# nnanhuang/S3Gaussian

Hardware: AMD Instinct MI355X
Metric: train_iters_per_sec (higher is better)
Workload: dtype f32

## Files before the change

### include/s3g_raster.h

```cpp
#ifndef S3G_RASTER_H
#define S3G_RASTER_H

#include <stddef.h>
#include <stdint.h>

#ifdef __cplusplus
extern "C" {
#endif

#define S3G_OK 0
#define S3G_ERR_INVALID_ARG 1
#define S3G_ERR_HIP 2
#define S3G_ERR_ALLOC 3
#define S3G_ERR_PREFILTERED 4

typedef void* (*s3g_resize_fn)(void* user, size_t bytes);

typedef struct s3g_raster_inputs {
  int P;
  int D;
  int M;
  int width, height;
  const float* background;
  const float* means3D;
// ... 14 lines not shown

int s3g_raster_forward(const s3g_raster_inputs* in,
                       s3g_resize_fn geometry_buffer, void* geometry_user,
                       s3g_resize_fn binning_buffer, void* binning_user,
                       s3g_resize_fn image_buffer, void* image_user,
                       float* out_color, float* out_depth, int* radii,
                       int* num_rendered, void* stream );

int s3g_raster_forward_reuse(const s3g_raster_inputs* in, int R, const void* geometry_arena, const void* binning_arena,
                             void* image_arena, float* out_color, float* out_depth, void* stream);

int s3g_raster_forward_decompose(const s3g_raster_inputs* in, int R, const void* geometry_arena, const void* binning_arena,
                                 const void* image_arena, const uint8_t* is_dynamic, const long long* class_counts,
                                 float* out_color_d, float* out_depth_d,
                                 float* out_color_s, float* out_depth_s, void* stream);

int s3g_raster_forward2(const s3g_raster_inputs* in, const float* colors2,
                        s3g_resize_fn geometry_buffer, void* geometry_user,
                        s3g_resize_fn binning_buffer, void* binning_user,
                        s3g_resize_fn image_buffer, void* image_user,
                        float* out_color, float* out_depth, float* out_color2, int* radii,
                        int* num_rendered, void* stream );

typedef struct s3g_raster_async {
  uint32_t capacity_instances;
  uint32_t capacity_slots;
  uint32_t sort_lds_keys;
  int long_lists;
  void* geometry_arena;
  void* binning_arena;
  void* image_arena;
  uint32_t* status_device;
  uint32_t* status_host;
  int forward_only;
  uint32_t* sticky_device;
  void* status_event;
} s3g_raster_async;
int s3g_raster_arena_bytes(int P, int width, int height, uint32_t capacity_instances, uint32_t capacity_slots,
                           size_t* geometry_bytes, size_t* binning_bytes, size_t* image_bytes);
int s3g_raster_forward_async(const s3g_raster_inputs* in, const float* colors2, const s3g_raster_async* async_,
                             float* out_color, float* out_depth, float* out_color2, int* radii, void* stream);

size_t s3g_raster_backward_workspace_bytes(int P, int R);
int s3g_raster_backward(const s3g_raster_inputs* in, int R, const int* radii,
                        const void* geometry_arena, const void* binning_arena, const void* image_arena,
                        void* workspace,
                        const float* dL_dpix, const float* dL_dpix_depth,
                        float* dL_dmean2D, float* dL_dconic, float* dL_dopacity, float* dL_dcolor,
                        float* dL_ddepth, float* dL_dmean3D, float* dL_dcov3D, float* dL_dsh,
                        float* dL_dscale, float* dL_drot, void* stream);

size_t s3g_raster_backward2_workspace_bytes(int P, int R);
int s3g_raster_backward2(const s3g_raster_inputs* in, const float* colors2, int R, const int* radii,
                         const void* geometry_arena, const void* binning_arena, const void* image_arena,
                         void* workspace,
                         const float* dL_dpix, const float* dL_dpix_depth, const float* dL_dpix2,
                         float* dL_dmean2D, float* dL_dconic, float* dL_dopacity, float* dL_dcolor, float* dL_dcolor2,
                         float* dL_ddepth, float* dL_dmean3D, float* dL_dcov3D, float* dL_dscale, float* dL_drot,
                         void* stream);

typedef struct s3g_densify_accum {
  float* xyz_gradient_accum;
  float* denom;
  float* max_radii2D;
} s3g_densify_accum;
int s3g_raster_backward_accum(const s3g_raster_inputs* in, int R, const int* radii,
                              const void* geometry_arena, const void* binning_arena, const void* image_arena,
                              void* workspace, const float* dL_dpix, const float* dL_dpix_depth,
                              float* dL_dmean2D, float* dL_dconic, float* dL_dopacity, float* dL_dcolor,
                              float* dL_ddepth, float* dL_dmean3D, float* dL_dcov3D, float* dL_dsh,
                              float* dL_dscale, float* dL_drot, const s3g_densify_accum* dens, void* stream);
int s3g_raster_backward2_accum(const s3g_raster_inputs* in, const float* colors2, int R, const int* radii,
                               const void* geometry_arena, const void* binning_arena, const void* image_arena,
                               void* workspace, const float* dL_dpix, const float* dL_dpix_depth, const float* dL_dpix2,
                               float* dL_dmean2D, float* dL_dconic, float* dL_dopacity, float* dL_dcolor,
                               float* dL_dcolor2, float* dL_ddepth, float* dL_dmean3D, float* dL_dcov3D,
                               float* dL_dscale, float* dL_drot, const s3g_densify_accum* dens, void* stream);

void s3g_raster_set_exact_cull(int on);
int s3g_raster_get_exact_cull(void);

int s3g_raster_set_backward_wave_bounds(int on);

int s3g_raster_set_bin_band(int tiles);

int s3g_mark_visible(int P, const float* means3D, const float* viewmatrix, const float* projmatrix,
                     uint8_t* present, void* stream);

enum {
  S3G_PROFILE_BLEND_FORWARD = 0,
  S3G_PROFILE_BLEND_BACKWARD = 1,
  S3G_PROFILE_HEXPLANE_FORWARD = 2,
  S3G_PROFILE_HEXPLANE_BACKWARD_POINT = 3,
  S3G_PROFILE_HEXPLANE_SCATTER = 4,
  S3G_PROFILE_MLP_FORWARD = 5,
  S3G_PROFILE_MLP_BACKWARD = 6,
  S3G_PROFILE_MLP_WGRAD = 7,
  S3G_PROFILE_ADAM = 8,
  S3G_PROFILE_DEFORM_INFER = 9,
  S3G_PROFILE_IDS = 10
};
void s3g_profile_enable(int on);
int s3g_profile_read(int id, double* total_ms, double* total_instances, double* total_pixels);

const char* s3g_last_error(void);

int s3g_abi_version(void);

#ifdef __cplusplus
}
#endif
#endif
```

### s3gaussian_amd/_lib.py

```python
from __future__ import annotations

import ctypes as C
import os
import subprocess

_HERE = os.path.dirname(os.path.abspath(__file__))
LIB_PATH = os.environ.get("S3G_LIB_PATH") or os.path.join(_HERE, "lib", "libs3g.so")
CSRC_DIR = os.path.join(_HERE, "csrc")

ABI_VERSION = 16

RESIZE_FN = C.CFUNCTYPE(C.c_void_p, C.c_void_p, C.c_size_t)


class RasterInputs(C.Structure):
    _fields_ = [
        ("P", C.c_int), ("D", C.c_int), ("M", C.c_int), ("width", C.c_int), ("height", C.c_int),
        ("background", C.c_void_p), ("means3D", C.c_void_p), ("shs", C.c_void_p), ("colors_precomp", C.c_void_p),
        ("opacities", C.c_void_p), ("scales", C.c_void_p), ("scale_modifier", C.c_float), ("rotations", C.c_void_p),
        ("cov3D_precomp", C.c_void_p), ("viewmatrix", C.c_void_p), ("projmatrix", C.c_void_p), ("cam_pos", C.c_void_p),
        ("tan_fovx", C.c_float), ("tan_fovy", C.c_float), ("prefiltered", C.c_int), ("debug", C.c_int),
    ]


# ... 39 lines not shown
    L.s3g_raster_backward.restype = C.c_int
    L.s3g_raster_backward.argtypes = [C.POINTER(RasterInputs), C.c_int] + [vp] * 18
    L.s3g_raster_backward_workspace_bytes.restype = C.c_size_t
    L.s3g_raster_backward_workspace_bytes.argtypes = [C.c_int, C.c_int]
    L.s3g_raster_forward2.restype = C.c_int
    L.s3g_raster_forward2.argtypes = [C.POINTER(RasterInputs), vp, RESIZE_FN, vp, RESIZE_FN, vp, RESIZE_FN, vp, vp, vp, vp, vp,
                                      C.POINTER(C.c_int), vp]
    L.s3g_raster_set_exact_cull.restype = None
    L.s3g_raster_set_exact_cull.argtypes = [C.c_int]
    L.s3g_raster_get_exact_cull.restype = C.c_int
    L.s3g_raster_backward2.restype = C.c_int
    L.s3g_raster_backward2.argtypes = [C.POINTER(RasterInputs), vp, C.c_int] + [vp] * 19
    L.s3g_raster_backward2_workspace_bytes.restype = C.c_size_t
    L.s3g_raster_backward2_workspace_bytes.argtypes = [C.c_int, C.c_int]
    L.s3g_mark_visible.restype = C.c_int
    L.s3g_mark_visible.argtypes = [C.c_int, vp, vp, vp, vp, vp]
    L.s3g_raster_forward_decompose.restype = C.c_int
    L.s3g_raster_forward_decompose.argtypes = [C.POINTER(RasterInputs), C.c_int] + [vp] * 10
    L.s3g_raster_backward_accum.restype = C.c_int
    L.s3g_raster_backward_accum.argtypes = [C.POINTER(RasterInputs), C.c_int] + [vp] * 17 + [C.POINTER(DensifyAccum), vp]
    L.s3g_raster_backward2_accum.restype = C.c_int
    L.s3g_raster_backward2_accum.argtypes = [C.POINTER(RasterInputs), vp, C.c_int] + [vp] * 18 + [C.POINTER(DensifyAccum), vp]
    L.s3g_raster_arena_bytes.restype = C.c_int
    L.s3g_raster_arena_bytes.argtypes = [C.c_int, C.c_int, C.c_int, C.c_uint32, C.c_uint32] + [C.POINTER(C.c_size_t)] * 3
    L.s3g_raster_forward_async.restype = C.c_int
    L.s3g_raster_forward_async.argtypes = [C.POINTER(RasterInputs), vp, C.POINTER(RasterAsync), vp, vp, vp, vp, vp]
    L.s3g_densify_stats.restype = C.c_int
    L.s3g_densify_stats.argtypes = [C.c_int, vp, C.c_int, vp, vp, vp, vp, vp, vp]
    L.s3g_densify_stats_guarded.restype = C.c_int
    L.s3g_densify_stats_guarded.argtypes = [C.c_int, vp, C.c_int, vp, vp, vp, vp, vp, vp, vp]
    _lib = L
    return L


def _bind_fast_paths():
    import torch
    raw = getattr(torch._C, "_cuda_getCurrentRawStream", None)
    cur = getattr(torch._C, "_cuda_getDevice", None)
    return torch, raw, cur


_torch = _raw_stream = _cur_device = None


def stream_ptr() -> int:
    global _torch, _raw_stream, _cur_device
    if _torch is None:
        _torch, _raw_stream, _cur_device = _bind_fast_paths()
    if _raw_stream is not None and _cur_device is not None:
        return _raw_stream(_cur_device())
    return _torch.cuda.current_stream().cuda_stream


class _NullContext:
    __slots__ = ()

    def __enter__(self):
        return None

    def __exit__(self, *exc):
        return False


_NULL = _NullContext()


def on_device(dev):
    global _torch, _raw_stream, _cur_device
    if _torch is None:
        _torch, _raw_stream, _cur_device = _bind_fast_paths()
    if _cur_device is not None and getattr(dev, "index", None) is not None and _cur_device() == dev.index:
        return _NULL
    return _torch.cuda.device(dev)


def check(code: int) -> None:
    if code != 0:
        msg = lib().s3g_last_error().decode("utf-8", "replace")
        if code == 1:
            raise Exception(msg)
        raise RuntimeError(f"libs3g error {code}: {msg}")


EXPORTED_SYMBOLS = ["s3g_raster_forward", "s3g_raster_forward_reuse", "s3g_raster_forward_decompose", "s3g_raster_forward2", "s3g_raster_forward_async", "s3g_raster_arena_bytes", "s3g_adam_step_guarded", "s3g_raster_backward", "s3g_raster_backward_workspace_bytes", "s3g_raster_backward2", "s3g_raster_backward2_workspace_bytes", "s3g_hexplane_forward_workspace_bytes", "s3g_knn_workspace_bytes", "s3g_knn_mean_dist2", "s3g_hexplane_forward", "s3g_hexplane_backward", "s3g_hexplane_backward_algo", "s3g_hexplane_backward_workspace_bytes", "s3g_hexplane_backward_scratch_rows", "s3g_hexplane_debug_walk_mask", "s3g_hexplane_set_deterministic", "s3g_hexplane_get_deterministic", "s3g_hexplane_sort_state_words", "s3g_profile_enable", "s3g_profile_read", "s3g_ssim_forward", "s3g_ssim_backward", "s3g_plane_regulation", "s3g_scale_unless_one", "s3g_pixel_losses_forward", "s3g_pixel_losses_combine", "s3g_pixel_losses_backward", "s3g_photometric_forward", "s3g_photometric_backward", "s3g_glue_forward", "s3g_glue_backward", "s3g_deform_mlp_forward", "s3g_deform_mlp_backward", "s3g_deform_mlp_backward_ordered", "s3g_deform_mlp_wgrad_partial_bytes", "s3g_deform_mlp_stash_bytes", "s3g_deform_mlp_pack_bytes", "s3g_deform_mlp_set_arithmetic", "s3g_deform_mlp_get_arithmetic", "s3g_deform_infer", "s3g_deform_infer_split", "s3g_deform_infer_workspace_bytes", "s3g_adam_step", "s3g_densify_stats", "s3g_densify_stats_guarded", "s3g_density_count_words", "s3g_density_classify_densify", "s3g_density_classify_prune", "s3g_density_scan", "s3g_density_apply", "s3g_density_reset_opacity", "s3g_image_metrics_workspace_bytes", "s3g_image_metrics", "s3g_scene_flow_workspace_bytes", "s3g_scene_flow_colors", "s3g_frame_workspace_bytes", "s3g_frame_tiles", "s3g_split_count_words", "s3g_split_workspace_bytes", "s3g_split_classify", "s3g_split_mask_offsets", "s3g_split_pack_rows", "s3g_lpips_weights_bytes", "s3g_lpips_pack_weights", "s3g_lpips_workspace_bytes", "s3g_lpips", "s3g_lpips_vgg_weights_bytes", "s3g_lpips_vgg_pack_weights", "s3g_lpips_vgg_workspace_bytes", "s3g_lpips_vgg", "s3g_raster_backward_accum", "s3g_raster_backward2_accum", "s3g_mark_visible", "s3g_raster_set_exact_cull", "s3g_raster_get_exact_cull", "s3g_raster_set_bin_band", "s3g_raster_set_backward_wave_bounds", "s3g_last_error", "s3g_abi_version"]
```

### s3gaussian_amd/csrc/raster_backward.hip

```cpp
#include "geom_math.hpp"
#include "raster_dev.hpp"

namespace s3g {

template <int CTRL, int ROW_MASK>
__device__ __forceinline__ float dpp_add(float v) {
  const int t = __builtin_amdgcn_update_dpp(0, __float_as_int(v), CTRL, ROW_MASK, 0xf, false);
  return v + __int_as_float(t);
}
__device__ __forceinline__ float wave_sum_lane63(float v) {
  v = dpp_add<0x111, 0xf>(v);
  v = dpp_add<0x112, 0xf>(v);
  v = dpp_add<0x114, 0xf>(v);
  v = dpp_add<0x118, 0xf>(v);
  v = dpp_add<0x142, 0xa>(v);
  v = dpp_add<0x143, 0xc>(v);
  return v;
}

__device__ __forceinline__ float row_sum_lane15(float v) {
  v = dpp_add<0x111, 0xf>(v);
  v = dpp_add<0x112, 0xf>(v);
  v = dpp_add<0x114, 0xf>(v);
  v = dpp_add<0x118, 0xf>(v);
  asm volatile("" : "+v"(v));
  return v;
}

#define S3G_DPP_SET(dst, src, ctrl, bank) \
  asm volatile("v_add_f32_dpp %0, %1, %1 " ctrl " row_mask:0xf bank_mask:" bank : "=v"(dst) : "v"(src))
#define S3G_DPP_ACC(dst, src, ctrl, bank) \
  asm volatile("v_add_f32_dpp %0, %1, %1 " ctrl " row_mask:0xf bank_mask:" bank : "+v"(dst) : "v"(src))
#define S3G_DPP_SELF(dst, ctrl) asm volatile("v_add_f32_dpp %0, %0, %0 " ctrl " row_mask:0xf bank_mask:0xf" : "+v"(dst))
template <int NV>
__device__ __forceinline__ void row_transpose_reduce(const float* v , float* q ) {
  static_assert(NV > 8 && NV <= 16, "values per visit");
  float r[8];
  asm volatile("s_nop 1");
#pragma unroll
  for (int i = 0; i < 8; i++) {
    S3G_DPP_SET(r[i], v[i], "row_ror:8", "0x3");
    if (i + 8 < NV) S3G_DPP_ACC(r[i], v[i + 8], "row_ror:8", "0xc");
  }
  asm volatile("s_nop 1");
#pragma unroll
  for (int i = 0; i < 4; i++) {
    S3G_DPP_SET(q[i], r[i], "row_half_mirror", "0x5");
    S3G_DPP_ACC(q[i], r[i + 4], "row_half_mirror", "0xa");
  }
  asm volatile("s_nop 1");
#pragma unroll
  for (int i = 0; i < 4; i++) S3G_DPP_SELF(q[i], "quad_perm:[1,0,3,2]");
  asm volatile("s_nop 1");
#pragma unroll
  for (int i = 0; i < 4; i++) S3G_DPP_SELF(q[i], "quad_perm:[2,3,0,1]");
}

template <int NX>
__global__ void __launch_bounds__(256)
blend_backward_kernel(int W, int H, int gx, int tiles, const uint2* __restrict__ ranges,
                      const uint32_t* __restrict__ tile_hi, const uint32_t* __restrict__ point_list,
                      const float* __restrict__ bg, const float2* __restrict__ means2D,
                      const float4* __restrict__ conic_opacity, const float* __restrict__ colors,
                      const float* __restrict__ depths, const float* __restrict__ final_Ts,
                      const uint32_t* __restrict__ n_contrib, const float* __restrict__ dL_dpixels,
                      const float* __restrict__ dL_dpixel_depths, float* __restrict__ records ,
                      const float* __restrict__ colors2, const float* __restrict__ dL_dpixels2, int wave_bounds) {
  constexpr uint32_t BATCH = 32;
  constexpr int NR = NX ? NREC + 4 : NREC;
  constexpr int SLOTS = 16;
  __shared__ StagedGaussian sg[BATCH];
  __shared__ float4 sg2[NX ? BATCH : 1];
  constexpr int NV = NX ? NREC + 3 : NREC;
  constexpr int RS = BATCH + 1;
  constexpr int SLOT_FLOATS = NV * RS;
  __shared__ float acc[SLOTS][SLOT_FLOATS];
  __shared__ uint32_t visited[4];

  const uint32_t tile = xcd_swizzle(blockIdx.x, gridDim.x);
  if (tile >= (uint32_t)tiles) return;
  const uint2 rg = ranges[tile];
  const uint32_t hi = tile_hi[tile] - rg.x;
  if (hi == 0) return;
  const int tx = tile % gx, ty = tile / gx;
  const int tid = threadIdx.x, lane = tid & 63, wave = tid >> 6;
  const int px = tx * TILE_X + (tid & 15), py = ty * TILE_Y + (tid >> 4);
  const bool inside = px < W && py < H;
  const float pxf = (float)px, pyf = (float)py;
  const size_t pix = (size_t)py * W + px, N = (size_t)H * W;

  const float T_final = inside ? final_Ts[pix] : 0.f;
  const uint32_t last_contributor = inside ? n_contrib[pix] : 0u;
  uint32_t whi = last_contributor;
  for (int off = 32; off >= 1; off >>= 1) whi = max(whi, (uint32_t)__shfl_xor((int)whi, off));
  whi = wave_bounds ? __builtin_amdgcn_readfirstlane(whi) : hi;
  float gr = 0.f, gg = 0.f, gb = 0.f, gd = 0.f;
  if (inside) {
    gr = dL_dpixels[pix];
    gg = dL_dpixels[N + pix];
    gb = dL_dpixels[2 * N + pix];
    gd = dL_dpixel_depths[pix];
  }
  float g2r = 0.f, g2g = 0.f, g2b = 0.f;
  if (NX && inside) {
    g2r = dL_dpixels2[pix];
    g2g = dL_dpixels2[N + pix];
    g2b = dL_dpixels2[2 * N + pix];
  }
  float bg_dot = bg[0] * gr + bg[1] * gg + bg[2] * gb;
  if (NX) bg_dot += bg[0] * g2r + bg[1] * g2g + bg[2] * g2b;

  float T = T_final;
  float ar = 0.f, ag = 0.f, ab = 0.f, ad = 0.f;
  float last_alpha = 0.f, lr = 0.f, lg = 0.f, lb = 0.f, ld = 0.f;
  float a2r = 0.f, a2g = 0.f, a2b = 0.f, l2r = 0.f, l2g = 0.f, l2b = 0.f;

  for (uint32_t done_cnt = 0; done_cnt < hi; done_cnt += BATCH) {
    const uint32_t cnt = min(BATCH, hi - done_cnt);
    __syncthreads();
    if ((uint32_t)tid < cnt) {
      const uint32_t pos = hi - 1 - (done_cnt + tid);
      const uint32_t id = point_list[rg.x + pos];
      const float2 mm = means2D[id];
      const float4 co = conic_opacity[id];
      StagedGaussian s;
      s.a = make_float4(mm.x, mm.y, -0.5f * LOG2E * co.x, -LOG2E * co.y);
      s.b = make_float4(-0.5f * LOG2E * co.z, co.w, depths[id], colors[3 * (size_t)id]);
      s.c = make_float4(colors[3 * (size_t)id + 1], colors[3 * (size_t)id + 2], 0.f, 0.f);
      sg[tid] = s;
      if (NX) sg2[tid] = make_float4(colors2[3 * (size_t)id], colors2[3 * (size_t)id + 1], colors2[3 * (size_t)id + 2], 0.f);
    }
    __syncthreads();

    const uint32_t j0 = hi - done_cnt > whi ? hi - done_cnt - whi : 0u;
    uint32_t vis = 0u;
    for (uint32_t j = j0; j < cnt; j++) {
      const uint32_t pos = hi - 1 - (done_cnt + j);
      bool valid = pos < last_contributor;
      const float4 A = sg[j].a;
      const float4 B = sg[j].b;
      const float dx = A.x - pxf, dy = A.y - pyf;
      const float q = gaussian_exponent2(dx, dy, A.z, A.w, B.x);
      const float G = __builtin_amdgcn_exp2f(q);
      const float alpha = fminf(0.99f, B.y * G);
      valid = valid && !(q > 0.f) && !(alpha < 1.0f / 255.0f);
      if (__ballot(valid) == 0ull) continue;
      vis |= 1u << j;

      float p_r = 0.f, p_g = 0.f, p_b = 0.f, p_d = 0.f, s0 = 0.f, sx = 0.f, sy = 0.f, sxx = 0.f, sxy = 0.f, syy = 0.f;
      float p2_r = 0.f, p2_g = 0.f, p2_b = 0.f;
      if (valid) {
        const float4 Cc = sg[j].c;
        const float cr = B.w, cg = Cc.x, cb = Cc.y, cd = B.z;
        const float rcp = __builtin_amdgcn_rcpf(1.f - alpha);
        T = T * rcp;
        const float w = alpha * T;
        const float one_m_la = 1.f - last_alpha;
        ar = last_alpha * lr + one_m_la * ar;
        ag = last_alpha * lg + one_m_la * ag;
        ab = last_alpha * lb + one_m_la * ab;
        ad = last_alpha * ld + one_m_la * ad;
        lr = cr; lg = cg; lb = cb; ld = cd;
        float dL_dalpha = (cr - ar) * gr + (cg - ag) * gg + (cb - ab) * gb + (cd - ad) * gd;
        if (NX) {
          const float4 C2 = sg2[j];
          a2r = last_alpha * l2r + one_m_la * a2r;
          a2g = last_alpha * l2g + one_m_la * a2g;
          a2b = last_alpha * l2b + one_m_la * a2b;
          l2r = C2.x; l2g = C2.y; l2b = C2.z;
          dL_dalpha += (C2.x - a2r) * g2r + (C2.y - a2g) * g2g + (C2.z - a2b) * g2b;
          p2_r = w * g2r; p2_g = w * g2g; p2_b = w * g2b;
        }
        dL_dalpha *= T;
        last_alpha = alpha;
        dL_dalpha += (-T_final * rcp) * bg_dot;
        p_r = w * gr; p_g = w * gg; p_b = w * gb; p_d = w * gd;
        const float v = dL_dalpha * G;
        const float vx = v * dx, vy = v * dy;
        s0 = v; sx = vx; sy = vy; sxx = vx * dx; sxy = vx * dy; syy = vy * dy;
      }
      const float vals[13] = {p_r, p_g, p_b, p_d, s0, sx, sy, sxx, sxy, syy, p2_r, p2_g, p2_b};
      float q4[4];
      row_transpose_reduce<NV>(vals, q4);
      if ((lane & 3) == 0) {
        float* aw = &acc[wave * 4 + (lane >> 4)][(lane & 12) * RS + j];
#pragma unroll
        for (int i = 0; i < 4; i++)
          if ((lane & 12) + i < NV) aw[i * RS] = q4[i];
      }
    }
    if (lane == 0) visited[wave] = vis;
    __syncthreads();
    const uint32_t g = (uint32_t)tid % BATCH, k = (uint32_t)tid / BATCH;
    if (k < NR / 2 && g < cnt) {
      uint32_t seen[4];
#pragma unroll
      for (int w = 0; w < 4; w++) seen[w] = 0u - ((visited[w] >> g) & 1u);
      auto slot = [&](int q, uint32_t v) { return __uint_as_float(__float_as_uint(acc[q][v * RS + g]) & seen[q / 4]); };
      const uint32_t v1 = 2 * k + 1 < (uint32_t)NV ? 2 * k + 1 : 2 * k;
      float lo = slot(0, 2 * k), hi2 = slot(0, v1);
#pragma unroll
      for (int q = 1; q < SLOTS; q++) {
        lo += slot(q, 2 * k);
        hi2 += slot(q, v1);
      }
      const uint32_t pos = hi - 1 - (done_cnt + g);
      float2* rec = reinterpret_cast<float2*>(records + (size_t)(rg.x + pos) * NR);
      rec[k] = make_float2(lo, 2 * k + 1 < (uint32_t)NV ? hi2 : 0.f);
    }
  }
}

struct GeomBwdArgs {
  int P, D, M;
  const float* means3D;
  const int* radii;
  const float* shs;
  const uint8_t* clamped;
  const float* scales;
  const float* rotations;
  float scale_modifier;
  const float* cov3Ds;
  const float* view;
  const float* proj;
  const float* campos;
  float fx, fy, tan_fovx, tan_fovy;
  int W, H, gx;
  const ushort4* rect;
  const uint32_t* gauss_off;
  const uint32_t* slot_pos;
  const uint32_t* tile_hi;
  const float* records;
  const float4* conic_opacity;
  const uint32_t* ctrl;
  float* dL_dmean2D;
  float* dL_dconic;
  float* dL_dopacity;
  float* dL_dcolor;
  float* dL_dcolor2;
  float* dL_ddepth;
  float* dL_dmean3D;
  float* dL_dcov3D;
  float* dL_dsh;
  float* dL_dscale;
  float* dL_drot;
  float* dens_accum;
  float* dens_denom;
  float* dens_max_radii;
};

#ifndef S3G_GATHER_BATCH
#define S3G_GATHER_BATCH 3
#endif
template <int NR>
__device__ __forceinline__ void gather_records(const GeomBwdArgs& a, const ushort4 r, uint32_t o, int k0, int stride,
                                               float* acc) {
  constexpr int B = S3G_GATHER_BATCH;
  const int w = (int)r.z - (int)r.x, n = w * ((int)r.w - (int)r.y);
  for (int k = k0; k < n; k += B * stride) {
    uint32_t pos[B], hi[B];
#pragma unroll
    for (int j = 0; j < B; j++) {
      const int kk = k + j * stride;
      const int kc = kk < n ? kk : k;
      const int ty = (int)r.y + kc / w, tx = (int)r.x + kc % w;
      pos[j] = a.slot_pos[o + kc];
      hi[j] = a.tile_hi[ty * a.gx + tx];
    }
    float2 v[B][NR / 2];
#pragma unroll
    for (int j = 0; j < B; j++) {
#pragma unroll
      for (int q = 0; q < NR / 2; q++) v[j][q] = make_float2(0.f, 0.f);
      if (k + j * stride < n && pos[j] < hi[j]) {
// ... 170 lines not shown
        DSH(1, -SH_C1 * y); DSH(2, SH_C1 * z); DSH(3, -SH_C1 * x);
        dRdx[ch] = -SH_C1 * SH(3); dRdy[ch] = -SH_C1 * SH(1); dRdz[ch] = SH_C1 * SH(2);
        if (deg > 1) {
          const float xx = x * x, yy = y * y, zz = z * z, xy = x * y, yz = y * z, xz = x * z;
          DSH(4, SH_C2[0] * xy); DSH(5, SH_C2[1] * yz); DSH(6, SH_C2[2] * (2.f * zz - xx - yy));
          DSH(7, SH_C2[3] * xz); DSH(8, SH_C2[4] * (xx - yy));
          dRdx[ch] += SH_C2[0] * y * SH(4) + SH_C2[2] * 2.f * -x * SH(6) + SH_C2[3] * z * SH(7) + SH_C2[4] * 2.f * x * SH(8);
          dRdy[ch] += SH_C2[0] * x * SH(4) + SH_C2[1] * z * SH(5) + SH_C2[2] * 2.f * -y * SH(6) + SH_C2[4] * 2.f * -y * SH(8);
          dRdz[ch] += SH_C2[1] * y * SH(5) + SH_C2[2] * 2.f * 2.f * z * SH(6) + SH_C2[3] * x * SH(7);
          if (deg > 2) {
            DSH(9, SH_C3[0] * y * (3.f * xx - yy)); DSH(10, SH_C3[1] * xy * z); DSH(11, SH_C3[2] * y * (4.f * zz - xx - yy));
            DSH(12, SH_C3[3] * z * (2.f * zz - 3.f * xx - 3.f * yy)); DSH(13, SH_C3[4] * x * (4.f * zz - xx - yy));
            DSH(14, SH_C3[5] * z * (xx - yy)); DSH(15, SH_C3[6] * x * (xx - 3.f * yy));
            dRdx[ch] += (SH_C3[0] * SH(9) * 3.f * 2.f * xy + SH_C3[1] * SH(10) * yz + SH_C3[2] * SH(11) * -2.f * xy +
                         SH_C3[3] * SH(12) * -3.f * 2.f * xz + SH_C3[4] * SH(13) * (-3.f * xx + 4.f * zz - yy) +
                         SH_C3[5] * SH(14) * 2.f * xz + SH_C3[6] * SH(15) * 3.f * (xx - yy));
            dRdy[ch] += (SH_C3[0] * SH(9) * 3.f * (xx - yy) + SH_C3[1] * SH(10) * xz + SH_C3[2] * SH(11) * (-3.f * yy + 4.f * zz - xx) +
                         SH_C3[3] * SH(12) * -3.f * 2.f * yz + SH_C3[4] * SH(13) * -2.f * xy + SH_C3[5] * SH(14) * -2.f * yz +
                         SH_C3[6] * SH(15) * -3.f * 2.f * xy);
            dRdz[ch] += (SH_C3[1] * SH(10) * xy + SH_C3[2] * SH(11) * 4.f * 2.f * yz + SH_C3[3] * SH(12) * 3.f * (2.f * zz - xx - yy) +
                         SH_C3[4] * SH(13) * 4.f * 2.f * xz + SH_C3[5] * SH(14) * (xx - yy));
          }
        }
      }
    }
#undef SH
#undef DSH
    const float ddx = dRdx[0] * dRGB[0] + dRdx[1] * dRGB[1] + dRdx[2] * dRGB[2];
    const float ddy = dRdy[0] * dRGB[0] + dRdy[1] * dRGB[1] + dRdy[2] * dRGB[2];
    const float ddz = dRdz[0] * dRGB[0] + dRdz[1] * dRGB[1] + dRdz[2] * dRGB[2];
    const float3 v = dir_orig;
    const float sum2 = v.x * v.x + v.y * v.y + v.z * v.z;
    const float invsum32 = 1.0f / sqrtf(sum2 * sum2 * sum2);
    dmx += ((+sum2 - v.x * v.x) * ddx - v.y * v.x * ddy - v.z * v.x * ddz) * invsum32;
    dmy += (-v.x * v.y * ddx + (sum2 - v.y * v.y) * ddy - v.z * v.y * ddz) * invsum32;
    dmz += (-v.x * v.z * ddx - v.y * v.z * ddy + (sum2 - v.z * v.z) * ddz) * invsum32;
  }
  a.dL_dmean3D[3 * (size_t)idx + 0] = dmx;
  a.dL_dmean3D[3 * (size_t)idx + 1] = dmy;
  a.dL_dmean3D[3 * (size_t)idx + 2] = dmz;

  if (a.scales != nullptr) {
    const float4 rot = reinterpret_cast<const float4*>(a.rotations)[idx];
    const float r = rot.x, x = rot.y, y = rot.z, z = rot.w;
    const M3 R = quat_to_R(rot);
    const float3 s = make_float3(a.scale_modifier * a.scales[3 * idx], a.scale_modifier * a.scales[3 * idx + 1],
                                 a.scale_modifier * a.scales[3 * idx + 2]);
    M3 S = {{{s.x, 0.f, 0.f}, {0.f, s.y, 0.f}, {0.f, 0.f, s.z}}};
    M3 Mm = m3_mul(S, R);
    M3 dSigma = {{{dcov[0], 0.5f * dcov[1], 0.5f * dcov[2]}, {0.5f * dcov[1], dcov[3], 0.5f * dcov[4]}, {0.5f * dcov[2], 0.5f * dcov[4], dcov[5]}}};
    M3 M2;
#pragma unroll
    for (int cc_ = 0; cc_ < 3; cc_++)
#pragma unroll
      for (int rr = 0; rr < 3; rr++) M2.m[cc_][rr] = 2.0f * Mm.m[cc_][rr];
    M3 dM = m3_mul(M2, dSigma);
    M3 Rt = m3_T(R), dMt = m3_T(dM);
    a.dL_dscale[3 * (size_t)idx + 0] = Rt.m[0][0] * dMt.m[0][0] + Rt.m[0][1] * dMt.m[0][1] + Rt.m[0][2] * dMt.m[0][2];
    a.dL_dscale[3 * (size_t)idx + 1] = Rt.m[1][0] * dMt.m[1][0] + Rt.m[1][1] * dMt.m[1][1] + Rt.m[1][2] * dMt.m[1][2];
    a.dL_dscale[3 * (size_t)idx + 2] = Rt.m[2][0] * dMt.m[2][0] + Rt.m[2][1] * dMt.m[2][1] + Rt.m[2][2] * dMt.m[2][2];
    const float sv[3] = {s.x, s.y, s.z};
#pragma unroll
    for (int k = 0; k < 3; k++)
#pragma unroll
      for (int rr = 0; rr < 3; rr++) dMt.m[k][rr] *= sv[k];
#define Dm(c_, r_) dMt.m[c_][r_]
    float4 dq;
    dq.x = 2 * z * (Dm(0, 1) - Dm(1, 0)) + 2 * y * (Dm(2, 0) - Dm(0, 2)) + 2 * x * (Dm(1, 2) - Dm(2, 1));
    dq.y = 2 * y * (Dm(1, 0) + Dm(0, 1)) + 2 * z * (Dm(2, 0) + Dm(0, 2)) + 2 * r * (Dm(1, 2) - Dm(2, 1)) - 4 * x * (Dm(2, 2) + Dm(1, 1));
    dq.z = 2 * x * (Dm(1, 0) + Dm(0, 1)) + 2 * r * (Dm(2, 0) - Dm(0, 2)) + 2 * z * (Dm(1, 2) + Dm(2, 1)) - 4 * y * (Dm(2, 2) + Dm(0, 0));
    dq.w = 2 * r * (Dm(0, 1) - Dm(1, 0)) + 2 * x * (Dm(2, 0) + Dm(0, 2)) + 2 * y * (Dm(1, 2) + Dm(2, 1)) - 4 * z * (Dm(1, 1) + Dm(0, 0));
#undef Dm
    reinterpret_cast<float4*>(a.dL_drot)[idx] = dq;
  } else {
    a.dL_dscale[i3] = a.dL_dscale[i3 + 1] = a.dL_dscale[i3 + 2] = 0.f;
    reinterpret_cast<float4*>(a.dL_drot)[idx] = make_float4(0.f, 0.f, 0.f, 0.f);
  }
}

}

using namespace s3g;

static bool g_wave_bounds = true;
extern "C" int s3g_raster_set_backward_wave_bounds(int on) {
  const int prev = g_wave_bounds ? 1 : 0;
  g_wave_bounds = on != 0;
  return prev;
}

extern "C" size_t s3g_raster_backward_workspace_bytes(int P, int R) {
  (void)P;
  return ((size_t)(R > 0 ? R : 0) * NREC * sizeof(float) + 127) & ~size_t(127);
}
extern "C" size_t s3g_raster_backward2_workspace_bytes(int P, int R) {
  (void)P;
  return ((size_t)(R > 0 ? R : 0) * (NREC + 4) * sizeof(float) + 127) & ~size_t(127);
}

template <int NX>
static int raster_backward_impl(const char* who, const s3g_raster_inputs* in, const float* colors2, int R, const int* radii,
                                const void* geometry_arena, const void* binning_arena, const void* image_arena,
                                void* workspace, const float* dL_dpix, const float* dL_dpix_depth, const float* dL_dpix2,
                                float* dL_dmean2D, float* dL_dconic, float* dL_dopacity, float* dL_dcolor,
                                float* dL_dcolor2, float* dL_ddepth, float* dL_dmean3D, float* dL_dcov3D, float* dL_dsh,
                                float* dL_dscale, float* dL_drot, const s3g_densify_accum* dens, void* stream_) {
  hipStream_t stream = (hipStream_t)stream_;
  if (dens && !(dens->xyz_gradient_accum && dens->denom && dens->max_radii2D)) {
    set_error("%s: s3g_densify_accum needs all three arrays", who);
    return S3G_ERR_INVALID_ARG;
  }
  if (!in) {
    set_error("%s: NULL inputs", who);
    return S3G_ERR_INVALID_ARG;
  }
  const int P = in->P, W = in->width, H = in->height;
  if (P == 0) return S3G_OK;
  if (!radii || !geometry_arena || !image_arena || (R > 0 && (!binning_arena || !workspace)) || !dL_dpix ||
      !dL_dpix_depth || !dL_dmean2D || !dL_dopacity || !dL_dcolor || !dL_dmean3D || !dL_dcov3D || !dL_dscale ||
      !dL_drot || (in->shs && !dL_dsh) || (NX && (!colors2 || !dL_dpix2 || !dL_dcolor2 || !in->colors_precomp))) {
    set_error("%s: NULL array argument", who);
    return S3G_ERR_INVALID_ARG;
  }
  const bool debug = in->debug != 0;
  const Arenas a = reopen_arenas(in, R, geometry_arena, binning_arena, image_arena);
  const int gx = a.gx, tiles = a.tiles;
  const GeomState& g = a.g;
  const ImageState& im = a.im;
  const BinningState& b = a.b;
  float* records = reinterpret_cast<float*>(workspace);

  const float* color_ptr = in->colors_precomp ? in->colors_precomp : g.rgb;
  if (R > 0) {
    const uint32_t tile_blocks = ((uint32_t)tiles + 7u) & ~7u;
    profile_begin(S3G_PROFILE_BLEND_BACKWARD, stream);
    hipLaunchKernelGGL(blend_backward_kernel<NX>, dim3(tile_blocks), dim3(256), 0, stream, W, H, gx, tiles, im.ranges,
                       im.tile_hi, b.point_list, in->background, g.means2D, g.conic_opacity, color_ptr, g.depths,
                       im.final_T, im.n_contrib, dL_dpix, dL_dpix_depth, records, colors2, dL_dpix2,
                       g_wave_bounds ? 1 : 0);
    profile_end(S3G_PROFILE_BLEND_BACKWARD, stream, (double)R, (double)W * H);
    S3G_KERNEL_CHECK(stream, debug);
  }
  GeomBwdArgs ga;
  ga.P = P; ga.D = in->D; ga.M = in->M; ga.means3D = in->means3D; ga.radii = radii; ga.shs = in->shs;
  ga.clamped = g.clamped; ga.scales = in->scales; ga.rotations = in->rotations; ga.scale_modifier = in->scale_modifier;
  ga.cov3Ds = in->cov3D_precomp ? in->cov3D_precomp : g.cov3D;
  ga.view = in->viewmatrix; ga.proj = in->projmatrix; ga.campos = in->cam_pos;
  ga.fy = H / (2.0f * in->tan_fovy); ga.fx = W / (2.0f * in->tan_fovx);
  ga.tan_fovx = in->tan_fovx; ga.tan_fovy = in->tan_fovy;
  ga.W = W; ga.H = H; ga.gx = gx;
  ga.rect = g.rect; ga.gauss_off = g.gauss_off; ga.slot_pos = b.slot_pos; ga.tile_hi = im.tile_hi;
  ga.records = records; ga.conic_opacity = g.conic_opacity; ga.ctrl = im.ctrl;
  ga.dL_dmean2D = dL_dmean2D; ga.dL_dconic = dL_dconic; ga.dL_dopacity = dL_dopacity; ga.dL_dcolor = dL_dcolor;
  ga.dL_dcolor2 = dL_dcolor2; ga.dL_ddepth = dL_ddepth;
  ga.dL_dmean3D = dL_dmean3D; ga.dL_dcov3D = dL_dcov3D; ga.dL_dsh = dL_dsh; ga.dL_dscale = dL_dscale; ga.dL_drot = dL_drot;
  ga.dens_accum = dens ? dens->xyz_gradient_accum : nullptr;
  ga.dens_denom = dens ? dens->denom : nullptr;
  ga.dens_max_radii = dens ? dens->max_radii2D : nullptr;
  hipLaunchKernelGGL(geometry_backward_kernel<NX>, dim3((P + 255) / 256), dim3(256), 0, stream, ga);
  S3G_KERNEL_CHECK(stream, debug);
  return S3G_OK;
}

extern "C" int s3g_raster_backward(const s3g_raster_inputs* in, int R, const int* radii, const void* geometry_arena,
                                   const void* binning_arena, const void* image_arena, void* workspace,
                                   const float* dL_dpix, const float* dL_dpix_depth, float* dL_dmean2D, float* dL_dconic,
                                   float* dL_dopacity, float* dL_dcolor, float* dL_ddepth, float* dL_dmean3D,
                                   float* dL_dcov3D, float* dL_dsh, float* dL_dscale, float* dL_drot, void* stream_) {
  return raster_backward_impl<0>("s3g_raster_backward", in, nullptr, R, radii, geometry_arena, binning_arena, image_arena,
                                 workspace, dL_dpix, dL_dpix_depth, nullptr, dL_dmean2D, dL_dconic, dL_dopacity, dL_dcolor,
                                 nullptr, dL_ddepth, dL_dmean3D, dL_dcov3D, dL_dsh, dL_dscale, dL_drot, nullptr, stream_);
}
extern "C" int s3g_raster_backward_accum(const s3g_raster_inputs* in, int R, const int* radii, const void* geometry_arena,
                                         const void* binning_arena, const void* image_arena, void* workspace,
                                         const float* dL_dpix, const float* dL_dpix_depth, float* dL_dmean2D,
                                         float* dL_dconic, float* dL_dopacity, float* dL_dcolor, float* dL_ddepth,
                                         float* dL_dmean3D, float* dL_dcov3D, float* dL_dsh, float* dL_dscale,
                                         float* dL_drot, const s3g_densify_accum* dens, void* stream_) {
  return raster_backward_impl<0>("s3g_raster_backward_accum", in, nullptr, R, radii, geometry_arena, binning_arena,
                                 image_arena, workspace, dL_dpix, dL_dpix_depth, nullptr, dL_dmean2D, dL_dconic, dL_dopacity,
                                 dL_dcolor, nullptr, dL_ddepth, dL_dmean3D, dL_dcov3D, dL_dsh, dL_dscale, dL_drot, dens,
                                 stream_);
}

extern "C" int s3g_raster_backward2(const s3g_raster_inputs* in, const float* colors2, int R, const int* radii,
                                    const void* geometry_arena, const void* binning_arena, const void* image_arena,
                                    void* workspace, const float* dL_dpix, const float* dL_dpix_depth,
                                    const float* dL_dpix2, float* dL_dmean2D, float* dL_dconic, float* dL_dopacity,
                                    float* dL_dcolor, float* dL_dcolor2, float* dL_ddepth, float* dL_dmean3D,
                                    float* dL_dcov3D, float* dL_dscale, float* dL_drot, void* stream_) {
  return raster_backward_impl<3>("s3g_raster_backward2", in, colors2, R, radii, geometry_arena, binning_arena, image_arena,
                                 workspace, dL_dpix, dL_dpix_depth, dL_dpix2, dL_dmean2D, dL_dconic, dL_dopacity, dL_dcolor,
                                 dL_dcolor2, dL_ddepth, dL_dmean3D, dL_dcov3D, nullptr, dL_dscale, dL_drot, nullptr, stream_);
}
extern "C" int s3g_raster_backward2_accum(const s3g_raster_inputs* in, const float* colors2, int R, const int* radii,
                                          const void* geometry_arena, const void* binning_arena, const void* image_arena,
                                          void* workspace, const float* dL_dpix, const float* dL_dpix_depth,
                                          const float* dL_dpix2, float* dL_dmean2D, float* dL_dconic, float* dL_dopacity,
                                          float* dL_dcolor, float* dL_dcolor2, float* dL_ddepth, float* dL_dmean3D,
                                          float* dL_dcov3D, float* dL_dscale, float* dL_drot,
                                          const s3g_densify_accum* dens, void* stream_) {
  return raster_backward_impl<3>("s3g_raster_backward2_accum", in, colors2, R, radii, geometry_arena, binning_arena,
                                 image_arena, workspace, dL_dpix, dL_dpix_depth, dL_dpix2, dL_dmean2D, dL_dconic, dL_dopacity,
                                 dL_dcolor, dL_dcolor2, dL_ddepth, dL_dmean3D, dL_dcov3D, nullptr, dL_dscale, dL_drot, dens,
                                 stream_);
}
```

### s3gaussian_amd/raster_C.py

```python
from __future__ import annotations

import ctypes as C
import os
import torch

from . import _lib

NUM_CHANNELS = 3


def _require_gpu(t: torch.Tensor, name: str) -> None:
    if not t.is_cuda:
        raise RuntimeError(f"{name} must live on the GPU (got {t.device}); the MI355X rasterizer has no CPU fallback")


def _f32(t: torch.Tensor, name: str) -> torch.Tensor:
    if t.numel() == 0:
        return t
    _require_gpu(t, name)
    if t.dtype != torch.float32:
        raise RuntimeError(f"{name} must be float32, got {t.dtype}")
    return t.contiguous()


# ... 467 lines not shown
    if P != 0:
        keep = [_f32(background, "bg"), _f32(means3D, "means3D"), _f32(sh, "sh"), _f32(colors, "colors_precomp"),
                _f32(scales, "scales"), _f32(rotations, "rotations"), _f32(cov3D_precomp, "cov3D_precomp"),
                _f32(viewmatrix, "viewmatrix"), _f32(projmatrix, "projmatrix"), _f32(campos, "campos"),
                _f32(dL_dout_color, "dL_dout_color"), _f32(dL_dout_depth, "dL_dout_depth"), radii.contiguous()]
        bg_, m3_, sh_, col_, sc_, rot_, cov_, view_, proj_, cam_, gcol_, gdep_, radii_ = keep
        inp = _inputs(P, degree, M, W, H, bg_, m3_, sh_, col_, None, sc_, scale_modifier, rot_, cov_, view_, proj_,
                      tan_fovx, tan_fovy, cam_, False, debug)
        work = torch.empty(L.s3g_raster_backward_workspace_bytes(P, int(R)), dtype=torch.uint8, device=dev)
        with _lib.on_device(dev):
            stream = _lib.stream_ptr()
            args = (C.byref(inp), int(R), radii_.data_ptr(), _ptr(geomBuffer), _ptr(binningBuffer),
                    _ptr(imageBuffer), _ptr(work), gcol_.data_ptr(), gdep_.data_ptr(),
                    v["means2D"].data_ptr(), _ptr(v["conic"]), v["opacity"].data_ptr(),
                    v["colors"].data_ptr(), _ptr(v["depths"]), v["means3D"].data_ptr(),
                    v["cov3D"].data_ptr(), _ptr(v["sh"]), v["scales"].data_ptr(), v["rot"].data_ptr())
            if densify_accum is None:
                code = L.s3g_raster_backward(*args, stream)
            else:
                code = L.s3g_raster_backward_accum(*args, C.byref(_densify_struct(densify_accum, P)), stream)
        _lib.check(code)
    out = (v["means2D"].view(P, 3), v["colors"].view(P, NUM_CHANNELS), v["opacity"].view(P, 1), v["means3D"].view(P, 3),
           v["cov3D"].view(P, 6), v["sh"].view(P, M, 3), v["scales"].view(P, 3), v["rot"].view(P, 4))
    if return_internals:
        out = out + (v["conic"].view(P, 2, 2), v["depths"].view(P, 1))
    return out


def rasterize_gaussians_backward2(background, means3D, radii, colors, colors2, scales, rotations, scale_modifier,
                                  cov3D_precomp, viewmatrix, projmatrix, tan_fovx, tan_fovy, dL_dout_color, dL_dout_depth,
                                  dL_dout_color2, campos, geomBuffer, R, binningBuffer, imageBuffer, debug, densify_accum=None):
    L = _lib.lib()
    dev = means3D.device
    P = means3D.size(0)
    H, W = dL_dout_color.size(1), dL_dout_color.size(2)
    v = _grad_slab(P, 0, dev, False)
    g_col2 = torch.empty((P, NUM_CHANNELS), dtype=torch.float32, device=dev)
    if P != 0:
        keep = [_f32(background, "bg"), _f32(means3D, "means3D"), _f32(colors, "colors_precomp"), _f32(colors2, "colors2"),
                _f32(scales, "scales"), _f32(rotations, "rotations"), _f32(cov3D_precomp, "cov3D_precomp"),
                _f32(viewmatrix, "viewmatrix"), _f32(projmatrix, "projmatrix"), _f32(campos, "campos"),
                _f32(dL_dout_color, "dL_dout_color"), _f32(dL_dout_depth, "dL_dout_depth"),
                _f32(dL_dout_color2, "dL_dout_color2"), radii.contiguous()]
        bg_, m3_, col_, col2_, sc_, rot_, cov_, view_, proj_, cam_, gcol_, gdep_, gcol2_, radii_ = keep
        inp = _inputs(P, 0, 0, W, H, bg_, m3_, None, col_, None, sc_, scale_modifier, rot_, cov_, view_, proj_,
                      tan_fovx, tan_fovy, cam_, False, debug)
        work = torch.empty(L.s3g_raster_backward2_workspace_bytes(P, int(R)), dtype=torch.uint8, device=dev)
        with _lib.on_device(dev):
            stream = _lib.stream_ptr()
            args = (C.byref(inp), col2_.data_ptr(), int(R), radii_.data_ptr(), _ptr(geomBuffer),
                    _ptr(binningBuffer), _ptr(imageBuffer), _ptr(work), gcol_.data_ptr(),
                    gdep_.data_ptr(), gcol2_.data_ptr(), v["means2D"].data_ptr(), None,
                    v["opacity"].data_ptr(), v["colors"].data_ptr(), g_col2.data_ptr(), None,
                    v["means3D"].data_ptr(), v["cov3D"].data_ptr(), v["scales"].data_ptr(),
                    v["rot"].data_ptr())
            if densify_accum is None:
                code = L.s3g_raster_backward2(*args, stream)
            else:
                code = L.s3g_raster_backward2_accum(*args, C.byref(_densify_struct(densify_accum, P)), stream)
        _lib.check(code)
    else:
        g_col2.zero_()
    return (v["means2D"].view(P, 3), v["colors"].view(P, NUM_CHANNELS), g_col2, v["opacity"].view(P, 1),
            v["means3D"].view(P, 3), v["cov3D"].view(P, 6), v["scales"].view(P, 3), v["rot"].view(P, 4))


def _densify_struct(acc, P) -> _lib.DensifyAccum:
    a, d, m = acc
    for name, t_ in (("xyz_gradient_accum", a), ("denom", d), ("max_radii2D", m)):
        if not (t_.is_cuda and t_.dtype == torch.float32 and t_.is_contiguous() and t_.numel() == P):
            raise RuntimeError(f"densify_accum: {name} must be a contiguous float32 GPU tensor with {P} elements")
    return _lib.DensifyAccum(a.data_ptr(), d.data_ptr(), m.data_ptr())


def set_exact_cull(on: bool) -> bool:
    global _geom_cache
    L = _lib.lib()
    prev = bool(L.s3g_raster_get_exact_cull())
    L.s3g_raster_set_exact_cull(int(bool(on)))
    _geom_cache = None
    return prev


def mark_visible(means3D, viewmatrix, projmatrix):
    L = _lib.lib()
    P = means3D.size(0)
    present = torch.zeros((P,), dtype=torch.bool, device=means3D.device)
    if P != 0:
        _require_gpu(means3D, "means3D")
        m3, view, proj = _f32(means3D, "means3D"), _f32(viewmatrix, "viewmatrix"), _f32(projmatrix, "projmatrix")
        with _lib.on_device(means3D.device):
            stream = _lib.stream_ptr()
            code = L.s3g_mark_visible(P, m3.data_ptr(), view.data_ptr(), proj.data_ptr(), present.data_ptr(), stream)
        _lib.check(code)
    return present
```

Before: 145.6.

## Double-buffer gaussian staging in blend backward to prefetch the next batch

Adds a double-buffered shared-memory staging path to the blend backward kernel. While the current batch is blended, the next batch's gaussian attributes are gathered into registers, then parked into the other LDS buffer after the compute loop, which removes one barrier per batch. The goal is to hide global-memory gather latency behind the blend math. It doubles staging LDS use and adds registers for the held values, which can lower occupancy. The new path is on by default and can be switched off through a new runtime setter.

After: 145.3 (median of 2 runs). No clear change (-0.2%).

```diff
diff --git a/include/s3g_raster.h b/include/s3g_raster.h
--- a/include/s3g_raster.h
+++ b/include/s3g_raster.h
@@ -120,6 +120,8 @@
 
 int s3g_raster_set_backward_wave_bounds(int on);
 
+int s3g_raster_set_backward_staging(int on);
+
 int s3g_raster_set_bin_band(int tiles);
 
 int s3g_mark_visible(int P, const float* means3D, const float* viewmatrix, const float* projmatrix,
diff --git a/s3gaussian_amd/_lib.py b/s3gaussian_amd/_lib.py
--- a/s3gaussian_amd/_lib.py
+++ b/s3gaussian_amd/_lib.py
@@ -145,4 +145,4 @@
         raise RuntimeError(f"libs3g error {code}: {msg}")
 
 
-EXPORTED_SYMBOLS = ["s3g_raster_forward", "s3g_raster_forward_reuse", "s3g_raster_forward_decompose", "s3g_raster_forward2", "s3g_raster_forward_async", "s3g_raster_arena_bytes", "s3g_adam_step_guarded", "s3g_raster_backward", "s3g_raster_backward_workspace_bytes", "s3g_raster_backward2", "s3g_raster_backward2_workspace_bytes", "s3g_hexplane_forward_workspace_bytes", "s3g_knn_workspace_bytes", "s3g_knn_mean_dist2", "s3g_hexplane_forward", "s3g_hexplane_backward", "s3g_hexplane_backward_algo", "s3g_hexplane_backward_workspace_bytes", "s3g_hexplane_backward_scratch_rows", "s3g_hexplane_debug_walk_mask", "s3g_hexplane_set_deterministic", "s3g_hexplane_get_deterministic", "s3g_hexplane_sort_state_words", "s3g_profile_enable", "s3g_profile_read", "s3g_ssim_forward", "s3g_ssim_backward", "s3g_plane_regulation", "s3g_scale_unless_one", "s3g_pixel_losses_forward", "s3g_pixel_losses_combine", "s3g_pixel_losses_backward", "s3g_photometric_forward", "s3g_photometric_backward", "s3g_glue_forward", "s3g_glue_backward", "s3g_deform_mlp_forward", "s3g_deform_mlp_backward", "s3g_deform_mlp_backward_ordered", "s3g_deform_mlp_wgrad_partial_bytes", "s3g_deform_mlp_stash_bytes", "s3g_deform_mlp_pack_bytes", "s3g_deform_mlp_set_arithmetic", "s3g_deform_mlp_get_arithmetic", "s3g_deform_infer", "s3g_deform_infer_split", "s3g_deform_infer_workspace_bytes", "s3g_adam_step", "s3g_densify_stats", "s3g_densify_stats_guarded", "s3g_density_count_words", "s3g_density_classify_densify", "s3g_density_classify_prune", "s3g_density_scan", "s3g_density_apply", "s3g_density_reset_opacity", "s3g_image_metrics_workspace_bytes", "s3g_image_metrics", "s3g_scene_flow_workspace_bytes", "s3g_scene_flow_colors", "s3g_frame_workspace_bytes", "s3g_frame_tiles", "s3g_split_count_words", "s3g_split_workspace_bytes", "s3g_split_classify", "s3g_split_mask_offsets", "s3g_split_pack_rows", "s3g_lpips_weights_bytes", "s3g_lpips_pack_weights", "s3g_lpips_workspace_bytes", "s3g_lpips", "s3g_lpips_vgg_weights_bytes", "s3g_lpips_vgg_pack_weights", "s3g_lpips_vgg_workspace_bytes", "s3g_lpips_vgg", "s3g_raster_backward_accum", "s3g_raster_backward2_accum", "s3g_mark_visible", "s3g_raster_set_exact_cull", "s3g_raster_get_exact_cull", "s3g_raster_set_bin_band", "s3g_raster_set_backward_wave_bounds", "s3g_last_error", "s3g_abi_version"]
+EXPORTED_SYMBOLS = ["s3g_raster_forward", "s3g_raster_forward_reuse", "s3g_raster_forward_decompose", "s3g_raster_forward2", "s3g_raster_forward_async", "s3g_raster_arena_bytes", "s3g_adam_step_guarded", "s3g_raster_backward", "s3g_raster_backward_workspace_bytes", "s3g_raster_backward2", "s3g_raster_backward2_workspace_bytes", "s3g_hexplane_forward_workspace_bytes", "s3g_knn_workspace_bytes", "s3g_knn_mean_dist2", "s3g_hexplane_forward", "s3g_hexplane_backward", "s3g_hexplane_backward_algo", "s3g_hexplane_backward_workspace_bytes", "s3g_hexplane_backward_scratch_rows", "s3g_hexplane_debug_walk_mask", "s3g_hexplane_set_deterministic", "s3g_hexplane_get_deterministic", "s3g_hexplane_sort_state_words", "s3g_profile_enable", "s3g_profile_read", "s3g_ssim_forward", "s3g_ssim_backward", "s3g_plane_regulation", "s3g_scale_unless_one", "s3g_pixel_losses_forward", "s3g_pixel_losses_combine", "s3g_pixel_losses_backward", "s3g_photometric_forward", "s3g_photometric_backward", "s3g_glue_forward", "s3g_glue_backward", "s3g_deform_mlp_forward", "s3g_deform_mlp_backward", "s3g_deform_mlp_backward_ordered", "s3g_deform_mlp_wgrad_partial_bytes", "s3g_deform_mlp_stash_bytes", "s3g_deform_mlp_pack_bytes", "s3g_deform_mlp_set_arithmetic", "s3g_deform_mlp_get_arithmetic", "s3g_deform_infer", "s3g_deform_infer_split", "s3g_deform_infer_workspace_bytes", "s3g_adam_step", "s3g_densify_stats", "s3g_densify_stats_guarded", "s3g_density_count_words", "s3g_density_classify_densify", "s3g_density_classify_prune", "s3g_density_scan", "s3g_density_apply", "s3g_density_reset_opacity", "s3g_image_metrics_workspace_bytes", "s3g_image_metrics", "s3g_scene_flow_workspace_bytes", "s3g_scene_flow_colors", "s3g_frame_workspace_bytes", "s3g_frame_tiles", "s3g_split_count_words", "s3g_split_workspace_bytes", "s3g_split_classify", "s3g_split_mask_offsets", "s3g_split_pack_rows", "s3g_lpips_weights_bytes", "s3g_lpips_pack_weights", "s3g_lpips_workspace_bytes", "s3g_lpips", "s3g_lpips_vgg_weights_bytes", "s3g_lpips_vgg_pack_weights", "s3g_lpips_vgg_workspace_bytes", "s3g_lpips_vgg", "s3g_raster_backward_accum", "s3g_raster_backward2_accum", "s3g_mark_visible", "s3g_raster_set_exact_cull", "s3g_raster_get_exact_cull", "s3g_raster_set_bin_band", "s3g_raster_set_backward_wave_bounds", "s3g_raster_set_backward_staging", "s3g_last_error", "s3g_abi_version"]
diff --git a/s3gaussian_amd/csrc/raster_backward.hip b/s3gaussian_amd/csrc/raster_backward.hip
--- a/s3gaussian_amd/csrc/raster_backward.hip
+++ b/s3gaussian_amd/csrc/raster_backward.hip
@@ -56,7 +56,10 @@
   for (int i = 0; i < 4; i++) S3G_DPP_SELF(q[i], "quad_perm:[2,3,0,1]");
 }
 
-template <int NX>
+typedef float f32x4 __attribute__((ext_vector_type(4)));
+__device__ __forceinline__ f32x4 lds_read4(const float4* p) { return *reinterpret_cast<const f32x4*>(p); }
+
+template <int NX, bool AHEAD>
 __global__ void __launch_bounds__(256)
 blend_backward_kernel(int W, int H, int gx, int tiles, const uint2* __restrict__ ranges,
                       const uint32_t* __restrict__ tile_hi, const uint32_t* __restrict__ point_list,
@@ -69,8 +72,9 @@
   constexpr uint32_t BATCH = 32;
   constexpr int NR = NX ? NREC + 4 : NREC;
   constexpr int SLOTS = 16;
-  __shared__ StagedGaussian sg[BATCH];
-  __shared__ float4 sg2[NX ? BATCH : 1];
+  constexpr int NSG = AHEAD ? 2 : 1;
+  __shared__ StagedGaussian sg[NSG][BATCH];
+  __shared__ float4 sg2[NSG][NX ? BATCH : 1];
   constexpr int NV = NX ? NREC + 3 : NREC;
   constexpr int RS = BATCH + 1;
   constexpr int SLOT_FLOATS = NV * RS;
@@ -115,30 +119,61 @@
   float last_alpha = 0.f, lr = 0.f, lg = 0.f, lb = 0.f, ld = 0.f;
   float a2r = 0.f, a2g = 0.f, a2b = 0.f, l2r = 0.f, l2g = 0.f, l2b = 0.f;
 
+  auto entry_id = [&](uint32_t e) { return point_list[rg.x + (hi - 1 - min(e, hi - 1))]; };
+  struct Gathered {
+    float2 mm;
+    float4 co;
+    float depth, r, g, b, r2, g2, b2;
+  };
+  auto gather = [&](uint32_t id) {
+    Gathered v;
+    v.mm = means2D[id];
+    v.co = conic_opacity[id];
+    v.depth = depths[id];
+    v.r = colors[3 * (size_t)id]; v.g = colors[3 * (size_t)id + 1]; v.b = colors[3 * (size_t)id + 2];
+    if (NX) { v.r2 = colors2[3 * (size_t)id]; v.g2 = colors2[3 * (size_t)id + 1]; v.b2 = colors2[3 * (size_t)id + 2]; }
+    return v;
+  };
+  auto park = [&](int half, const Gathered& v) {
+    StagedGaussian s;
+    s.a = make_float4(v.mm.x, v.mm.y, -0.5f * LOG2E * v.co.x, -LOG2E * v.co.y);
+    s.b = make_float4(-0.5f * LOG2E * v.co.z, v.co.w, v.depth, v.r);
+    s.c = make_float4(v.g, v.b, 0.f, 0.f);
+    sg[half][tid] = s;
+    if (NX) sg2[half][tid] = make_float4(v.r2, v.g2, v.b2, 0.f);
+  };
+  const bool stager = (uint32_t)tid < BATCH;
+  const uint32_t slot = stager ? (uint32_t)tid : 0u;
+  uint32_t id_next = 0u;
+  if (AHEAD) {
+    id_next = entry_id(BATCH + slot);
+    if (stager) park(0, gather(entry_id(tid)));
+    __builtin_amdgcn_s_waitcnt(0x0f70);
+  }
+
   for (uint32_t done_cnt = 0; done_cnt < hi; done_cnt += BATCH) {
     const uint32_t cnt = min(BATCH, hi - done_cnt);
+    const int cur = AHEAD ? (int)(done_cnt / BATCH) & 1 : 0;
     __syncthreads();
-    if ((uint32_t)tid < cnt) {
-      const uint32_t pos = hi - 1 - (done_cnt + tid);
-      const uint32_t id = point_list[rg.x + pos];
-      const float2 mm = means2D[id];
-      const float4 co = conic_opacity[id];
-      StagedGaussian s;
-      s.a = make_float4(mm.x, mm.y, -0.5f * LOG2E * co.x, -LOG2E * co.y);
-      s.b = make_float4(-0.5f * LOG2E * co.z, co.w, depths[id], colors[3 * (size_t)id]);
-      s.c = make_float4(colors[3 * (size_t)id + 1], colors[3 * (size_t)id + 2], 0.f, 0.f);
-      sg[tid] = s;
-      if (NX) sg2[tid] = make_float4(colors2[3 * (size_t)id], colors2[3 * (size_t)id + 1], colors2[3 * (size_t)id + 2], 0.f);
-    }
-    __syncthreads();
+    if (!AHEAD) {
+      if ((uint32_t)tid < cnt) park(0, gather(entry_id(done_cnt + tid)));
+      __syncthreads();
+    }
+    Gathered ahead;
+    if (AHEAD) {
+      ahead = gather(id_next);
+      id_next = entry_id(done_cnt + 2 * BATCH + slot);
+    }
+    const StagedGaussian* sgc = sg[cur];
+    const float4* sg2c = sg2[cur];
 
     const uint32_t j0 = hi - done_cnt > whi ? hi - done_cnt - whi : 0u;
     uint32_t vis = 0u;
     for (uint32_t j = j0; j < cnt; j++) {
       const uint32_t pos = hi - 1 - (done_cnt + j);
       bool valid = pos < last_contributor;
-      const float4 A = sg[j].a;
-      const float4 B = sg[j].b;
+      const f32x4 A = lds_read4(&sgc[j].a);
+      const f32x4 B = lds_read4(&sgc[j].b);
       const float dx = A.x - pxf, dy = A.y - pyf;
       const float q = gaussian_exponent2(dx, dy, A.z, A.w, B.x);
       const float G = __builtin_amdgcn_exp2f(q);
@@ -150,7 +185,7 @@
       float p_r = 0.f, p_g = 0.f, p_b = 0.f, p_d = 0.f, s0 = 0.f, sx = 0.f, sy = 0.f, sxx = 0.f, sxy = 0.f, syy = 0.f;
       float p2_r = 0.f, p2_g = 0.f, p2_b = 0.f;
       if (valid) {
-        const float4 Cc = sg[j].c;
+        const f32x4 Cc = lds_read4(&sgc[j].c);
         const float cr = B.w, cg = Cc.x, cb = Cc.y, cd = B.z;
         const float rcp = __builtin_amdgcn_rcpf(1.f - alpha);
         T = T * rcp;
@@ -163,7 +198,7 @@
         lr = cr; lg = cg; lb = cb; ld = cd;
         float dL_dalpha = (cr - ar) * gr + (cg - ag) * gg + (cb - ab) * gb + (cd - ad) * gd;
         if (NX) {
-          const float4 C2 = sg2[j];
+          const f32x4 C2 = lds_read4(&sg2c[j]);
           a2r = last_alpha * l2r + one_m_la * a2r;
           a2g = last_alpha * l2g + one_m_la * a2g;
           a2b = last_alpha * l2b + one_m_la * a2b;
@@ -190,6 +225,10 @@
       }
     }
     if (lane == 0) visited[wave] = vis;
+    if (AHEAD) {
+      __builtin_amdgcn_s_waitcnt(0x0f70);
+      if (stager) park(cur ^ 1, ahead);
+    }
     __syncthreads();
     const uint32_t g = (uint32_t)tid % BATCH, k = (uint32_t)tid / BATCH;
     if (k < NR / 2 && g < cnt) {
@@ -526,6 +565,13 @@
 
 using namespace s3g;
 
+static bool g_staging = true;
+extern "C" int s3g_raster_set_backward_staging(int on) {
+  const int prev = g_staging ? 1 : 0;
+  g_staging = on != 0;
+  return prev;
+}
+
 static bool g_wave_bounds = true;
 extern "C" int s3g_raster_set_backward_wave_bounds(int on) {
   const int prev = g_wave_bounds ? 1 : 0;
@@ -578,10 +624,10 @@
   if (R > 0) {
     const uint32_t tile_blocks = ((uint32_t)tiles + 7u) & ~7u;
     profile_begin(S3G_PROFILE_BLEND_BACKWARD, stream);
-    hipLaunchKernelGGL(blend_backward_kernel<NX>, dim3(tile_blocks), dim3(256), 0, stream, W, H, gx, tiles, im.ranges,
-                       im.tile_hi, b.point_list, in->background, g.means2D, g.conic_opacity, color_ptr, g.depths,
-                       im.final_T, im.n_contrib, dL_dpix, dL_dpix_depth, records, colors2, dL_dpix2,
-                       g_wave_bounds ? 1 : 0);
+    auto* const blend = g_staging ? blend_backward_kernel<NX, true> : blend_backward_kernel<NX, false>;
+    hipLaunchKernelGGL(blend, dim3(tile_blocks), dim3(256), 0, stream, W, H, gx, tiles, im.ranges, im.tile_hi, b.point_list,
+                       in->background, g.means2D, g.conic_opacity, color_ptr, g.depths, im.final_T, im.n_contrib, dL_dpix,
+                       dL_dpix_depth, records, colors2, dL_dpix2, g_wave_bounds ? 1 : 0);
     profile_end(S3G_PROFILE_BLEND_BACKWARD, stream, (double)R, (double)W * H);
     S3G_KERNEL_CHECK(stream, debug);
   }
diff --git a/s3gaussian_amd/raster_C.py b/s3gaussian_amd/raster_C.py
--- a/s3gaussian_amd/raster_C.py
+++ b/s3gaussian_amd/raster_C.py
@@ -573,6 +573,13 @@
     return prev
 
 
+def set_backward_staging(on: bool) -> bool:
+    L = _lib.lib()
+    L.s3g_raster_set_backward_staging.restype = C.c_int
+    L.s3g_raster_set_backward_staging.argtypes = [C.c_int]
+    return bool(L.s3g_raster_set_backward_staging(int(bool(on))))
+
+
 def mark_visible(means3D, viewmatrix, projmatrix):
     L = _lib.lib()
     P = means3D.size(0)
```
